# netneurolab/pypyls

Hardware: AMD Instinct MI355X
Metric: resamples/sec (perm+boot), behavioral_pls X(500x200000)/Y(500x50) fp64 (higher is better)
Workload: dtype f64

## Files before the change

pypyls_amd/csrc/plsx_compact.hip:

```cpp
#include "plsx_internal.h"

using namespace plsxi;

namespace plsxi {

template <int MT, int KT, bool TAIL = false>
int launch_xprod_cboot(plsx_ctx* ctx, int nres, int nks_c, SplitEpi se, hipStream_t st)
{
    const size_t lds = compact_lds_bytes(MT, KT, 3, nks_c, se.npairs);
    HIPCHK(set_lds(k_xprod_compact<MT, KT, 3, TAIL>, lds));
    const int ncolblk = ceil_div(ctx->Bpad, 128);
    KTimer tm(ctx, KC_XPROD, st);
    hipLaunchKernelGGL((k_xprod_compact<MT, KT, 3, TAIL>), dim3(round_up(ncolblk, 8) * round_up(nres, 8)), dim3(256),
                       lds, st, ptr<double>(ctx->Afrag_c), (size_t)nks_c * MT * 64, ptr<double>(ctx->Xc), ctx->Bpad, nks_c,
                       ptr<double>(ctx->R), ctx->Bpad, ctx->Tpp, ptr<int>(ctx->out_row_c), ptr<int>(ctx->mom_idx_c),
                       (const double*)nullptr, nres, ncolblk, se);
    LAUNCHCHK();
    return 0;
}

int launch_cboot(plsx_ctx* ctx, int nres, int nks_c, SplitEpi se, hipStream_t st)
{
    const int MTc = ceil_div(ctx->Tp, 16);
    const bool tail = ctx->Tp - (MTc - 1) * 16 <= 4 && MTc >= 2;
    switch (MTc) {
        case 1: return launch_xprod_cboot<1, 12>(ctx, nres, nks_c, se, st);
        case 2: return tail ? launch_xprod_cboot<2, 6, true>(ctx, nres, nks_c, se, st)
                            : launch_xprod_cboot<2, 6>(ctx, nres, nks_c, se, st);
        case 3: return tail ? launch_xprod_cboot<3, 4, true>(ctx, nres, nks_c, se, st)
                            : launch_xprod_cboot<3, 4>(ctx, nres, nks_c, se, st);
        case 4: return tail ? launch_xprod_cboot<4, PLSX_CKT, true>(ctx, nres, nks_c, se, st)
                            : launch_xprod_cboot<4, PLSX_CKT>(ctx, nres, nks_c, se, st);
#define PLSX_CB(M, K) case M: return tail ? launch_xprod_cboot<M, K, true>(ctx, nres, nks_c, se, st) \
                                          : launch_xprod_cboot<M, K>(ctx, nres, nks_c, se, st);
        PLSX_CB(5, 2) PLSX_CB(6, 2) PLSX_CB(7, 1) PLSX_CB(8, 1) PLSX_CB(9, 1) PLSX_CB(10, 1) PLSX_CB(11, 1) PLSX_CB(12, 1) PLSX_CB(13, 1)
#undef PLSX_CB
        default: return fail(ctx, PLSX_ERR_STATE, "compact bootstrap blocks: T' > 208");
    }
}
// ... 46 lines not shown
```

pypyls_amd/csrc/plsx_core.hip:

```cpp
#include "plsx_internal.h"
#include "plsx_resample.h"
using namespace plsxi;

namespace plsxi {

const char* const kKernelClassNames[KC_COUNT] = {"k_xprod", "k_gram", "k_small", "k_urot", "k_nt_gemm",
                                                 "k_ucorr_partial", "k_simpls_dual", "k_build_A", "k_xprod_moments",
                                                 "k_sd_cv_score", "k_sd_coef", "k_coef_prod", "k_percentile", "k_contrast"};

int plan_groups(plsx_ctx* c)
{
    c->scaled = (c->method == PLSX_BEHAVIORAL && !c->cov) ? 1 : 0;
    c->momrows = (c->method == PLSX_BEHAVIORAL && (!c->cov || c->cv_mom)) ? 1 : 0;
    const int Jw = c->momrows ? c->J : 0;
    c->gps = 0;
    c->h_slice_row0.clear(); c->h_slice_rows.clear(); c->h_slice_cell0.clear(); c->h_slice_ncell.clear();
    auto fit = [&](int mt) {
        int b = 0;
        for (int n = 1; n <= 512; ++n) {
            int td = ceil_div(n * c->Tp, 16), tw = Jw ? ceil_div(n * Jw, 16) : 0;
            if (td + 2 * tw <= mt && tw * 16 <= 48) b = n; else break;
        }
        return b;
    };
// ... 1194 lines not shown
try {
    plsx_ctx* ctx = const_cast<plsx_ctx*>(cctx);
    if (!ctx || !out || cap < 1) return PLSX_ERR_ARG;
    double ms = 0.0;
    int launches = 0;
    for (auto& ev : ctx->events) {
        if (ev.cls != KC_XPROD) continue;
        float t = 0.f;
        if (hipEventSynchronize(ev.e1) == hipSuccess && hipEventElapsedTime(&t, ev.e0, ev.e1) == hipSuccess)
            ms += t;
        ++launches;
    }
    double crows = 0.0;
    if (ctx->last_compact_n > 0) {
        std::vector<int> cnt(ctx->last_compact_n);
        if (hipMemcpy(cnt.data(), ptr<int>(ctx->rowtab_c) + (size_t)ctx->last_compact_n * ctx->last_compact_ktot,
                      cnt.size() * sizeof(int), hipMemcpyDeviceToHost) == hipSuccess) {
            for (int c : cnt) crows += 4.0 * ((std::max(c, 1) + 3) / 4);
            crows /= (double)cnt.size() * ctx->S;
        }
    }
    const bool cmp = ctx->last_compact_n > 0;
    const auto uvar = [&](int nks) { return (double)(nks > 0 && ctx->urot_tail_l ? nks + 100 : nks); };
    double vals[21] = {ms, (double)launches, (double)(cmp ? 1 : (ctx->sepmom_used ? ctx->npg_d : ctx->npg)),
                       (double)(cmp ? ceil_div(ctx->Tp, 16) : (ctx->sepmom_used ? ctx->MTd : ctx->MT)),
                       (double)ctx->Gcap * ctx->npg, (double)ctx->timed_units, (double)use_dual(ctx), crows,
                       ctx->nt_flops, (double)ctx->quad_series, (double)ctx->quad_MT, (double)ctx->quad_gpl,
                       (double)ctx->urot_waves_l, (double)ctx->urot_splits_l, (double)ctx->urot_rps_l,
                       uvar(ctx->urot_nks_first), (double)ctx->gram_chunks_l, uvar(ctx->urot_nks_last),
                       (double)ctx->gram_kind_l, (double)ctx->split_blocks_l, (double)ctx->split_reader_l};
    int n = std::min(cap, 21);
    for (int i = 0; i < n; ++i) out[i] = vals[i];
    return n;
} PLSX_CATCH(const_cast<plsx_ctx*>(cctx))

int plsx_kernel_timing(const plsx_ctx* cctx, int kernel_class, double* ms_out, int* launches_out)
try {
    plsx_ctx* ctx = const_cast<plsx_ctx*>(cctx);
    if (!ctx || kernel_class < 0 || kernel_class >= KC_COUNT) return PLSX_ERR_ARG;
    double ms = 0.0;
    int launches = 0;
    for (auto& ev : ctx->events) {
        if (ev.cls != kernel_class) continue;
        float t = 0.f;
        if (hipEventSynchronize(ev.e1) == hipSuccess && hipEventElapsedTime(&t, ev.e0, ev.e1) == hipSuccess)
            ms += t;
        ++launches;
    }
    if (ms_out) *ms_out = ms;
    if (launches_out) *launches_out = launches;
    return PLSX_OK;
} PLSX_CATCH(const_cast<plsx_ctx*>(cctx))

const char* plsx_kernel_class_name(int kernel_class)
// ... 146 lines not shown
```

pypyls_amd/csrc/plsx_internal.h:

```cpp
#pragma once
#include "plsx_kernels.h"
#include <chrono>
#include "../../include/plsx.h"

#include <algorithm>
#include <cmath>
#include <cstdio>
#include <cstdlib>
#include <cstring>
#include <new>
#include <stdexcept>
#include <string>
#include <thread>
#include <vector>

struct Buf {
    void* p = nullptr;
    size_t bytes = 0;
};

enum {
    OPT_NO_REFINE = 0, OPT_MIN_BATCH, OPT_INBLOCK_MOMENTS, OPT_NO_COMPACT_BOOT, OPT_COMPACT_BOOT_ALWAYS,
    OPT_SEPMOM_ALWAYS, OPT_NO_GRAM4, OPT_UROT_GENERIC, OPT_UROT_NO_TAIL4, OPT_NO_FIXED_X, OPT_NO_DUAL_PERM,
    OPT_TWO_PASS_BOOT, OPT_SPLIT_INBLOCK, OPT_NO_SPLIT_FUSE, OPT_SPLIT_TWO_READERS, OPT_EXPECT_RESAMPLES,
    OPT_SIMPLS_JACOBI, OPT_PERCENTILE_SORT, OPT_QUAD_SUMS, OPT_SPLIT_READER8, OPT_SIMPLS_GLOBAL,
    OPT_CROSSCOV_SPARSE, OPT_COUNT
};
static const char* const kOptionNames[OPT_COUNT] = {
    "no_refine", "min_batch", "inblock_moments", "no_compact_boot", "compact_boot_always",
    "sepmom_always", "no_gram4", "urot_generic", "urot_no_tail4", "no_fixed_x", "no_dual_perm",
    "two_pass_boot", "split_inblock", "no_split_fuse", "split_two_readers", "expect_resamples",
    "simpls_jacobi", "percentile_sort", "quad_sums", "split_reader8", "simpls_global",
    "crosscov_sparse"};

#ifndef PLSX_CKT
#define PLSX_CKT 3
#endif

struct plsx_ctx {
    int device = 0;
    std::string err;
    int opt[OPT_COUNT] = {};
    bool has_data = false, has_orig = false;
    int method = 0, S = 0, B = 0, T = 0, J = 0, n_groups = 0, n_cond = 1, mc = 0, cov = 0;
    int Tp = 0, Tpp = 0, L = 0, Kpad = 0, nks = 0, Bx = 0, Bpad = 0;
    int MT = 24, npg = 0, w0 = 0, sq0 = 0, nmom_pad = 0, scaled = 0, momrows = 0, Gcap = 0, Galloc = 0;
    int nks_t = 0, LT = 0, cv_mom = 0;
    int afrag_group0 = 0;
    int sepmom = 0, MTd = 0, npg_d = 0, sepmom_used = 0;
    size_t group_stride_d = 0;
    Buf out_row_d, mom_idx_d, Afrag_m, momn_m, scale;
    Buf Afrag_c, rank_c, rowtab_c, m1_c, m2_c, out_row_c, mom_idx_c, mask_c;
    int has_compact_maps = 0;
    size_t group_stride = 0;
    int gps = 0;
    Buf row_slice, row_local, slice_cell0, cell_momrow;
// ... 42 lines not shown
    double* keepA = nullptr;
    long long keep_cap = 0, keep_n = 0;
    Buf cichunk;
    double* vipG = nullptr;
    long long vip_cap = 0, vip_n = 0;
    int vip_c = 0;
    int cperm_active = 0, cperm_c = 0, cperm_std = 0;
    const double* cperm_obs = nullptr;
    int* cperm_count = nullptr;
    double* cperm_max = nullptr;
    long long cperm_cap = 0, cperm_n = 0;
    Buf cpA, cppart, colsd;
    bool has_okx = false, has_oky = false;
    int n_okx = 0;
    double* mom_out_arg = nullptr;
    int ncomp = 0;
    int timing = 0;
    struct TimedEv { int cls; hipEvent_t e0, e1; };
    std::vector<TimedEv> events;
    long long timed_units = 0;
    double nt_flops = 0.0;
    int quad_MT = 0, quad_gpl = 0, quad_series = 0;
    int last_compact_n = 0, last_compact_ktot = 0;
    int urot_waves_l = 0, urot_splits_l = 0, urot_rps_l = 0;
    int urot_nks_first = 0, urot_nks_last = 0, urot_tail_l = 0;
    int gram_chunks_l = 0, gram_kind_l = 0;
    double scratch_gb = 48.0;
    long long R_geom[6] = {0, 0, 0, 0, 0, 0};
    size_t R_zeroed_bytes = 0;
    double map_ms_per_gb = 0.0;
    int scratch_fixed = 0;
    double last_ms = 0.0;
    int last_launches = 0;
    void* comm = nullptr;
    int comm_rank = 0, comm_world = 1;
    int comm_team = 0;
};

namespace plsxi {


inline int fail(plsx_ctx* c, int code, const std::string& msg)
{
    if (c) c->err = msg;
    return code;
}
// ... 127 lines not shown
int run_contrast_norms(plsx_ctx* ctx, int nres, double* out_sv, hipStream_t st);
int run_contrast_fill(plsx_ctx* ctx, int nres, hipStream_t st);
int run_percentile(plsx_ctx* ctx, const double* d_data, long long nseries, int n, int i_lo, double g_lo, int i_hi,
                   double g_hi, double* d_lo, double* d_hi, hipStream_t st);
inline void coef_close(plsx_ctx* ctx)
{
    ctx->coef_active = 0; ctx->coef_n = 0;
    ctx->keepA = nullptr; ctx->keep_cap = 0; ctx->keep_n = 0;
}
inline void vip_close(plsx_ctx* ctx)
{
    ctx->vipG = nullptr; ctx->vip_cap = 0; ctx->vip_n = 0; ctx->vip_c = 0;
}
inline void cperm_close(plsx_ctx* ctx)
{
    ctx->cperm_active = 0; ctx->cperm_c = 0; ctx->cperm_std = 0;
    ctx->cperm_obs = nullptr; ctx->cperm_count = nullptr; ctx->cperm_max = nullptr;
    ctx->cperm_cap = 0; ctx->cperm_n = 0;
}
int launch_xprod(plsx_ctx* ctx, int groups, hipStream_t st);
int launch_xprod_acc(plsx_ctx* ctx, const double* Afrag, size_t gstride, int groups, int L, hipStream_t st);
int run_xprod_fixed(plsx_ctx* ctx, const int* ysrc, int nres, hipStream_t st, const double* ystack);
MomLayout moment_layout(const plsx_ctx* ctx, int npairs);
int launch_moment_blocks_raw(plsx_ctx* ctx, const MomLayout& ml, SplitEpi se, hipStream_t st);
int ensure_compact_maps(plsx_ctx* ctx);
int run_xprod(plsx_ctx* ctx, const int* xsrc, const int* ysrc, int nres, hipStream_t st,
              bool prebuilt = false, const double* ystack = nullptr, long long ystride = -1, bool sparse_rows = false);
int launch_xprod_split(plsx_ctx* ctx, int groups, SplitEpi se, hipStream_t st);
int quad_finish(plsx_ctx* ctx, double* d_usum, double* d_usq, hipStream_t st, const QuadSet* qs = nullptr);
inline int quad_blocks(int tiles) { return tiles >= 8 ? ceil_div(tiles, 8) : 1; }
int launch_cboot(plsx_ctx* ctx, int nres, int nks_c, SplitEpi se, hipStream_t st);
int launch_csplit(plsx_ctx* ctx, int m, int nks_c, SplitEpi se, hipStream_t st, bool raw = false);
int run_nt(plsx_ctx* ctx, const double* A, long long strideA, int lda, int Ma,
           const double* B1, long long strideB1, int ldb1, int N1,
           const double* B2, long long strideB2, int ldb2, int N2, int K, int batch,
           double* C1, long long strideC1, int ldc1, double* C2, long long strideC2, int ldc2,
           hipStream_t st, bool sym = false, bool accumulate = false, bool one_chunk = false);
bool nt_sym_fits(int S);
int nt_strips(plsx_ctx* ctx, const double* A, int lda, int Ma, const double* Bm, int ldb, int N, int Kc,
              double* C, int ldc, hipStream_t st, bool one_chunk = false);
int form_gram_K(plsx_ctx* ctx, const double* X, int ldx, int S, int Kc, double* K, int ldk, hipStream_t st);
int run_dual_gp(plsx_ctx* ctx, int m, int Sd, const double* ScT, int L, hipStream_t st);
int run_gram_ex(plsx_ctx* ctx, int nres, int mode, const double* E, int Erows, double* Pout,
                hipStream_t st, const double* Rsrc = nullptr);
int run_gram(plsx_ctx* ctx, int nres, bool with_p, hipStream_t st);
int run_small(plsx_ctx* ctx, SmallArgs a, int nres, hipStream_t st, const double* Rref = nullptr);
// ... 13 lines not shown
```

pypyls_amd/csrc/plsx_k_prep.h:

```cpp
#pragma once
#include "plsx_common.h"


static __global__ void k_colmean(const double* __restrict__ X, int S, int B, double* __restrict__ mean)
{
    int b = blockIdx.x * blockDim.x + threadIdx.x;
    if (b >= B) return;
    double s = 0.0;
    for (int i = 0; i < S; ++i) s += X[(size_t)i * B + b];
    mean[b] = s / (double)S;
}

static __global__ void k_center_pad(const double* __restrict__ X, const double* __restrict__ mean,
                             int S, int B, double* __restrict__ Xc, int ldx)
{
    int b = blockIdx.x * blockDim.x + threadIdx.x;
    int i = blockIdx.y;
    if (b >= B || i >= S) return;
    Xc[(size_t)i * ldx + b] = X[(size_t)i * B + b] - mean[b];
}

static __global__ void k_cell_scale(const double* __restrict__ Xc, int ldx, int B, int J,
                             const int* __restrict__ cell_start, const int* __restrict__ cell_len,
                             double* __restrict__ Xn)
// ... 21 lines not shown
struct GroupLayout {
    int n;
    int Tp;
    int J;
    int T;
    int MT;
    int w0;
    int sq0;
    int Tpp;
    int gps = 0;
    const int* row_slice = nullptr;
    const int* row_local = nullptr;
    const int* slice_cell0 = nullptr;
};

static __global__ void k_build_A_behav(const double* __restrict__ Y0, long long y_stride, int T, int S,
                                const int* __restrict__ cell_start, const int* __restrict__ cell_len,
                                const int* __restrict__ xsrc, const int* __restrict__ ysrc,
                                GroupLayout lay, int covariance, int scaled,
                                double* __restrict__ Afrag, size_t group_stride,
                                double* __restrict__ mom_n, int nmom_pad, int dense_ld = 0,
                                double* __restrict__ Amom = nullptr, size_t mom_stride = 0,
                                const int* __restrict__ rank = nullptr, int mom_pairs = PLSX_MOM_PAIRS,
                                int chain_cap = 0)
{
    extern __shared__ double sm_b[];
    const int r = blockIdx.x, j = blockIdx.y;
    const int g = r / lay.n, rr = r % lay.n;
    const double* Y = Y0 + (size_t)r * y_stride;
    const int start = cell_start[j], len = cell_len[j];
    const int* xs = xsrc ? xsrc + (size_t)r * S : nullptr;
    const int* ys = ysrc ? ysrc + (size_t)r * S : nullptr;
    double* mean = sm_b;
    double* rstd = sm_b + T;
    __shared__ int s_cnt;
    const int tid = threadIdx.x;

    if (tid == 0) {
        int c = 0;
        for (int p = start; p < start + len; ++p) c += (xs ? xs[p] : p) >= 0;
        s_cnt = c;
    }
    __syncthreads();
    const int cnt = s_cnt;
    for (int t = tid; t < T; t += blockDim.x) {
        double s = 0.0;
        for (int p = start; p < start + len; ++p) {
// ... 71 lines not shown
            double c = 0.0;
            for (int q = pl; q >= 0; q = nxt[q]) c += 1.0;
            *d0 = c; *d1 = c;
        } else if (unique) { *d0 = 1.0; *d1 = 1.0; }
        else { atomicAdd(d0, 1.0); atomicAdd(d1, 1.0); }
    };
    if (scaled && sliced) {
        const int sa = lay.row_slice[j * T], sb = lay.row_slice[j * T + T - 1];
        for (int sl = sa; sl <= sb; ++sl) {
            const size_t gg = (size_t)r * lay.gps + sl;
            double* As = Afrag + gg * group_stride;
            const int mrow = j - lay.slice_cell0[sl];
            for (int pl = tid; pl < len; pl += blockDim.x) {
                int p = start + pl;
                int xi = xs ? xs[p] : p;
                if (xi < 0) continue;
                put_weight(As + afrag_off(lay.w0 * 16 + mrow, xi, lay.MT), As + afrag_off(lay.sq0 * 16 + mrow, xi, lay.MT), pl);
            }
            if (tid == 0) mom_n[gg * nmom_pad + mrow] = (double)cnt;
        }
    } else if (scaled && Amom) {
        const int pair = r * lay.J + j;
        double* Am = Amom + (size_t)(pair / mom_pairs) * mom_stride;
        const int mrow = pair % mom_pairs, mmt = mom_pairs / 8;
        for (int pl = tid; pl < len; pl += blockDim.x) {
            int p = start + pl;
            int xi = xs ? xs[p] : p;
            if (xi < 0) continue;
            put_weight(Am + afrag_off(mrow, xi, mmt), Am + afrag_off(mom_pairs + mrow, xi, mmt), pl);
        }
        if (tid == 0) mom_n[pair] = (double)cnt;
    } else if (scaled) {
        for (int pl = tid; pl < len; pl += blockDim.x) {
            int p = start + pl;
            int xi = xs ? xs[p] : p;
            if (xi < 0) continue;
            int mrow = rr * lay.J + j;
            put_weight(A + afrag_off(lay.w0 * 16 + mrow, xi, lay.MT), A + afrag_off(lay.sq0 * 16 + mrow, xi, lay.MT), pl);
        }
        if (tid == 0) mom_n[(size_t)g * nmom_pad + rr * lay.J + j] = (double)cnt;
    }
}

static __global__ void k_build_A_mc(int S, int J, int n_cond, int mean_centering,
                             const int* __restrict__ cell_of_pos,
                             const int* __restrict__ xsrc, GroupLayout lay,
                             double* __restrict__ Afrag, size_t group_stride, int dense_ld = 0, int chain_cap = 0)
{
    extern __shared__ int sm_mc[];
    __shared__ int cnt[PLSX_MAX_CELLS];
    const int r = blockIdx.x;
    const int g = r / lay.n, rr = r % lay.n;
// ... 290 lines not shown
```

pypyls_amd/csrc/plsx_k_xprod.h:

```cpp
#pragma once
#include <type_traits>
#include <utility>

template <class F, int... I>
__device__ __forceinline__ void xprod_static_for(F&& f, std::integer_sequence<int, I...>)
{
    (f(std::integral_constant<int, I>()), ...);
}
#include "plsx_common.h"
#include "plsx_k_prep.h"

#define PLSX_RSRC_FLAGS 0x00020000
template <int NT, int PASSES, bool EVEN, int STAGE>
__device__ __forceinline__ void stage_copy_buf(const double* src, double* dst, int tid, int wave)
{
    __amdgpu_buffer_rsrc_t rs = __builtin_amdgcn_make_buffer_rsrc((void*)src, (short)0, 0x7fffffff,
                                                                   PLSX_RSRC_FLAGS);
    const int voff = tid * 16;
#pragma unroll
    for (int p = 0; p < PASSES; ++p) {
        if (EVEN || p * NT + wave * 64 < STAGE / 2) {
            __builtin_amdgcn_raw_ptr_buffer_load_lds(
                rs, (__attribute__((address_space(3))) void*)(dst + (size_t)(p * NT + wave * 64) * 2),
                16, voff, p * NT * 16, 0, 0);
// ... 96 lines not shown
            const double b = xb[s];
            const double bsq = (NSQ > 0) ? b * b : 0.0;
#pragma unroll
            for (int m = 0; m < NA; ++m)
                acc[m] = mfma_f64(sA[(s * MT + m) * 64], (m < MT - NSQ) ? b : bsq, acc[m]);
        }
#pragma unroll
        for (int s = 0; s < KT; ++s) xb[s] = xn[s];
        __syncthreads();
    };
    int kt_first = 0;
    if constexpr (EPI == 7) {
        xprod_static_for([&](auto mm) {
#pragma unroll
            for (int j = 0; j < 4 / KT; ++j) {
                const int kt = (4 / KT) * decltype(mm)::value + j;
                if (kt < nkt) pass(kt, std::integral_constant<int, decltype(mm)::value + 1>());
            }
        }, std::make_integer_sequence<int, MT>());
        kt_first = min(nkt, 4 * MT / KT);
    }
    for (int kt = kt_first; kt < nkt; ++kt) pass(kt, std::integral_constant<int, MT>());

    constexpr int W0 = MT - 2 * NSQ, SQ0 = MT - NSQ, NMOM = NSQ * 16;
    if constexpr (EPI == 6) {
        static_assert(MT == 2 * NSQ, "EPI 6 is a moment-only instantiation");
#pragma unroll
        for (int j = 0; j < NSQ; ++j)
#pragma unroll
            for (int i = 0; i < 4; ++i) {
                const int pair = grp * (NSQ * 16) + j * 16 + kq + 4 * i;
                if (pair >= se.npairs || col >= ldr) continue;
                se.scale[(size_t)pair * ldr + col] = acc[j][i];
                se.scale2[(size_t)pair * ldr + col] = acc[NSQ + j][i];
            }
        return;
    }
    if constexpr (EPI == 4) {
        static_assert(MT == 2 * NSQ, "EPI 4 is the moment-only instantiation");
#pragma unroll
        for (int j = 0; j < NSQ; ++j)
#pragma unroll
            for (int i = 0; i < 4; ++i) {
                const int pair = grp * (NSQ * 16) + j * 16 + kq + 4 * i;
                if (pair >= se.npairs || col >= ldr) continue;
                const double m1 = acc[j][i], m2 = acc[NSQ + j][i];
                const double nn = mom_n[pair];
// ... 212 lines not shown
        for (int i = 0; i < 4; ++i)
            if (orow[i] >= 0) Rg[(size_t)orow[i] * ldr] = acc[m][i] * sc[i];
    }
}

__device__ __forceinline__ d2 load_x2_buf(const double* base, int voff)
{
    __amdgpu_buffer_rsrc_t rs = __builtin_amdgcn_make_buffer_rsrc((void*)base, (short)0, 0x7fffffff, PLSX_RSRC_FLAGS);
    return __builtin_bit_cast(d2, __builtin_amdgcn_raw_buffer_load_b128(rs, voff, 0, 0));
}

__host__ __device__ constexpr int compact_stage_lds(int MT, int KT) { return ((KT * MT * 64 + 127) / 128) * 128; }
__host__ __device__ constexpr int compact_scale_regs(int KT) { return KT < 4 ? KT : 4; }
__host__ __device__ constexpr size_t compact_lds_bytes(int MT, int KT, int EPI, int nks, int J)
{
    const size_t loop = (size_t)MT * 16 * 8 + (size_t)2 * compact_stage_lds(MT, KT) * 8 + (size_t)nks * 4 * 4;
    if (EPI == 3) return loop + (J > compact_scale_regs(KT) ? (size_t)J * 128 * 8 : 0);
    const size_t epi5 = (size_t)MT * 16 * 8 + (size_t)5 * J * 128 * 8 + (size_t)MT * 16 * 5 * 8;
    return EPI == 5 && epi5 > loop ? epi5 : loop;
}

__host__ __device__ constexpr int compact_waves(int MT, int EPI, bool TAIL)
{
    if (EPI == 3) return MT > 10 ? 2 : MT == 10 ? (TAIL ? 3 : 2) : MT > 6 ? 3 : MT > 4 ? 4 : (MT == 4 && TAIL) ? 5 : 4;
    return (EPI == 5 && MT == 4 && !TAIL) ? 3 : 4;
}

template <int MT, int KT, int EPI, bool TAIL>
__global__ __launch_bounds__(256, compact_waves(MT, EPI, TAIL))
void k_xprod_compact(const double* __restrict__ Afrag, size_t group_stride,
                     const double* __restrict__ X, int ldx, int nks,
                     double* __restrict__ R, int ldr, int rows_per_group,
                     const int* __restrict__ out_row, const int* __restrict__ mom_idx,
                     const double* __restrict__ mom_n, int n_groups, int ncolblk, SplitEpi se)
{
    static_assert(EPI == 3 || EPI == 5 || EPI == 8, "compact blocks: bootstrap (3), fused split-half (5) or raw first-half sums (8)");
    extern __shared__ __attribute__((aligned(16))) double smem[];
    constexpr int NW = 4, NT = NW * 64, BC = NW * 32;
    constexpr int STAGE = KT * MT * 64;
    constexpr int STAGE_LDS = compact_stage_lds(MT, KT);
    constexpr int PASSES = (STAGE + NT * 2 - 1) / (NT * 2);
    constexpr bool EVEN = (STAGE % (NT * 2)) == 0;
    constexpr int MF = TAIL ? MT - 1 : MT;
    constexpr int NSCR = compact_scale_regs(KT);
    static_assert(MT * 16 <= NT, "the row maps are staged by one thread per row");
    const int ncb = (ncolblk + 7) & ~7;
    const int sweep = blockIdx.x / (8 * ncb);
    const int within = blockIdx.x - sweep * (8 * ncb);
    const int slot = within >> 3;
    const int grp = sweep * 8 + (slot & 7);
    const int colblk = (slot >> 3) * 8 + (within & 7);
    if (grp >= n_groups || colblk >= ncolblk) return;
    const double* Ag = Afrag + (size_t)grp * group_stride;
    const int swave = __builtin_amdgcn_readfirstlane((int)threadIdx.x >> 6);

    d4 acc0[MF > 0 ? MF : 1], acc1[MF > 0 ? MF : 1];
#pragma unroll
    for (int m = 0; m < MF; ++m) { acc0[m] = (d4){0.0, 0.0, 0.0, 0.0}; acc1[m] = (d4){0.0, 0.0, 0.0, 0.0}; }
    double tl0 = 0.0, tl1 = 0.0;

    int* s_out = reinterpret_cast<int*>(smem);
    int* s_mom = s_out + MT * 16;
    double* sStage = smem + MT * 16;
    int* s_tab = reinterpret_cast<int*>(sStage + 2 * STAGE_LDS);
    const int J3 = se.npairs;
    double* sW = reinterpret_cast<double*>(s_tab + nks * 4) + swave * (J3 * 32);
    d2 scr[NSCR];
    {
    const int tid = threadIdx.x, lane = tid & 63, wave = tid >> 6;
    const int kq = lane >> 4;
    const int cw = wave * 32 + 2 * (lane & 15);
    const int col = colblk * BC + cw;
    const bool live = col < ldr;
    const int lcol8 = (live ? col : 0) * 8;
    const int toff = (lane & 48) + (lane & 3) - lane;

    const int* tabg = se.row_tab + (size_t)grp * nks * 4;
    const int ldx8 = ldx * 8;
    int row0[KT];
#pragma unroll
    for (int s = 0; s < KT; ++s) row0[s] = tabg[s * 4 + kq];
    stage_copy_buf<NT, PASSES, EVEN, STAGE>(Ag, sStage, tid, swave);
    int orw = -1, mix = -1;
    if (tid < MT * 16) {
        orw = out_row[tid];
        if (EPI != 8) mix = mom_idx[tid];
    }
    const int ksteps = max(1, (se.row_cnt[grp] + 3) >> 2);
    const int nkt = (ksteps + KT - 1) / KT;
    const int ntab = nkt * KT * 4;
// ... 47 lines not shown
                acc1[m] = mfma_f64(a, b1, acc1[m]);
            }
            if constexpr (TAIL) {
                const double a = sT[(s * MT + MT - 1) * 64];
                tl0 = mfma_f64_4x4(a, b0, tl0);
                tl1 = mfma_f64_4x4(a, b1, tl1);
            }
        }
    };
    const int* tp = s_tab + KT * 4 + kq;
    const double* An = Ag + STAGE;
    auto pass = [&](auto curc, const d2 (&xc)[KT], d2 (&xn)[KT]) {
        constexpr int CUR = decltype(curc)::value;
        stage_copy_buf<NT, PASSES, EVEN, STAGE>(An, sStage + (CUR ^ 1) * STAGE_LDS, tid, swave);
#pragma unroll
        for (int s = 0; s < KT; ++s) xn[s] = load_x2_buf(X, tp[s * 4] + lcol8);
        An += STAGE;
        tp += KT * 4;
        contract(curc, xc, std::true_type(), KT);
        __syncthreads();
    };
    auto last = [&](int cur, const d2 (&xc)[KT]) {
#pragma unroll
        for (int j = 0; j < NSCR; ++j) scr[j] = (d2){1.0, 1.0};
        if constexpr (EPI == 3) {
            if (J3 <= NSCR) {
#pragma unroll
                for (int j = 0; j < NSCR; ++j)
                    if (j < J3)
                        scr[j] = *reinterpret_cast<const d2*>(
                            reinterpret_cast<const char*>(se.scale + ((size_t)grp * J3 + j) * ldr) + lcol8);
            } else if (live) {
                __amdgpu_buffer_rsrc_t rs = __builtin_amdgcn_make_buffer_rsrc(
                    (void*)(se.scale + (size_t)grp * J3 * ldr + colblk * BC + swave * 32), (short)0, 0x7fffffff, PLSX_RSRC_FLAGS);
                const int ln4 = __lane_id() * 4;
                for (int j = 0; j < J3; ++j)
                    __builtin_amdgcn_raw_ptr_buffer_load_lds(
                        rs, (__attribute__((address_space(3))) void*)(sW + j * 32), 4, ln4, j * ldr * 8, 0, 0);
            }
        }
        contract(cur, xc, std::false_type(), ksteps - (nkt - 1) * KT);
        if constexpr (EPI == 5) __syncthreads();
    };
    {
        std::integral_constant<int, 0> c0;
        std::integral_constant<int, 1> c1;
        int kt = 0, cur = 0;
        for (; kt + 2 < nkt; kt += 2) { pass(c0, xa, xb); pass(c1, xb, xa); }
        if (kt + 1 < nkt) {
            pass(c0, xa, xb);
#pragma unroll
            for (int s = 0; s < KT; ++s) xa[s] = xb[s];
            cur = 1;
        }
        last(cur, xa);
    }
    }

    int tid16 = threadIdx.x * 16;
    if constexpr (EPI != 5) asm volatile("" : "+v"(tid16));
    const int tid = tid16 >> 4, lane = tid & 63, wave = tid >> 6, kq = lane >> 4;
    const int cw = wave * 32 + 2 * (lane & 15), col = colblk * BC + cw;
    const bool live = col < ldr;
    auto val0 = [&](int m, int i) -> double { return (TAIL && m == MT - 1) ? tl0 : acc0[m < MF ? m : 0][i]; };
    auto val1 = [&](int m, int i) -> double { return (TAIL && m == MT - 1) ? tl1 : acc1[m < MF ? m : 0][i]; };

    if constexpr (EPI == 8) {
        if (!live) return;
        double* Rg = R + (size_t)grp * rows_per_group * ldr + col;
#pragma unroll
        for (int m = 0; m < MT; ++m)
#pragma unroll
            for (int i = 0; i < 4; ++i) {
                if (TAIL && m == MT - 1 && i > 0) break;
                const int orow = s_out[m * 16 + kq + 4 * i];
                if (orow < 0) continue;
                __builtin_nontemporal_store((d2){val0(m, i), val1(m, i)}, reinterpret_cast<d2*>(&Rg[(size_t)orow * ldr]));
            }
        return;
// ... 108 lines not shown
```

pypyls_amd/csrc/plsx_xprod.hip:

```cpp
#include "plsx_internal.h"

using namespace plsxi;

namespace plsxi {

template <int MT, int NW, int KT, int NSQ>
int launch_xprod_t(plsx_ctx* ctx, int groups, hipStream_t st)
{
    const size_t stage = (size_t)2 * (((size_t)KT * MT * 64 + 127) / 128) * 128 * 8;
    const size_t epi = (size_t)NW * 2 * NSQ * 16 * 16 * 8 + (size_t)2 * MT * 16 * 4;
    const size_t lds = std::max(stage, epi);
    HIPCHK(set_lds(k_xprod<MT, NW, KT, NSQ>, lds));
    const int ncolblk = ctx->Bpad / (NW * 16);
    dim3 grid(ncolblk * round_up(groups, 8)), block(NW * 64);
    KTimer tm(ctx, KC_XPROD, st);
    hipLaunchKernelGGL((k_xprod<MT, NW, KT, NSQ>), grid, block, lds, st,
                       ptr<double>(ctx->Afrag) + (size_t)ctx->afrag_group0 * ctx->group_stride, ctx->group_stride,
                       ptr<double>(ctx->Xc), ctx->Bpad,
                       ctx->nks, ptr<double>(ctx->R), ctx->Bpad, ctx->npg * ctx->Tpp,
                       ptr<int>(ctx->out_row), ptr<int>(ctx->mom_idx), ptr<double>(ctx->mom_n),
                       std::max(ctx->nmom_pad, 0), groups, ncolblk, ctx->mom_out_arg,
                       SplitEpi{nullptr, nullptr, nullptr, nullptr, nullptr, 0, 0}, std::max(ctx->gps, 1));
    LAUNCHCHK();
    return 0;
// ... 32 lines not shown
        hipLaunchKernelGGL((k_xprod<MT, NW, KT, 0, 2>), dim3(ncolblk * round_up(groups, 8)), dim3(NW * 64), lds, st,
                           Afrag, gstride, ptr<double>(ctx->Xc), ctx->Bpad, ctx->nks, (double*)nullptr, ctx->Bpad, 0,
                           ptr<int>(ctx->out_row_w), (const int*)nullptr, (const double*)nullptr, 0, groups, ncolblk,
                           (double*)nullptr, se, 1);
    } else {
        constexpr int NW = 4;
        const size_t lds = std::max(stage, ((size_t)2 * L + 32) * PLSX_ACC_PITCH * 8 + (size_t)MT * 16 * 4);
        HIPCHK(set_lds(k_xprod<MT, NW, KT, 0, 2>, lds));
        const int ncolblk = ctx->Bpad / (NW * 16);
        hipLaunchKernelGGL((k_xprod<MT, NW, KT, 0, 2>), dim3(ncolblk * round_up(groups, 8)), dim3(NW * 64), lds, st,
                           Afrag, gstride, ptr<double>(ctx->Xc), ctx->Bpad, ctx->nks, (double*)nullptr, ctx->Bpad, 0,
                           ptr<int>(ctx->out_row_w), (const int*)nullptr, (const double*)nullptr, 0, groups, ncolblk,
                           (double*)nullptr, se, 1);
    }
    LAUNCHCHK();
    return 0;
}

static int stage_ksteps(int nks) { return nks % 3 == 0 ? 3 : (nks % 2 == 0 ? 2 : 1); }

template <int MT, int NW, int KT, int EPI>
int launch_moments_t(plsx_ctx* ctx, size_t stride, int groups, SplitEpi se, hipStream_t st)
{
    const size_t lds = (size_t)2 * (((size_t)KT * MT * 64 + 127) / 128) * 128 * 8;
    HIPCHK(set_lds(k_xprod<MT, NW, KT, MT / 2, EPI>, lds));
    const int ncolblk = ceil_div(ctx->Bpad, NW * 16);
    hipLaunchKernelGGL((k_xprod<MT, NW, KT, MT / 2, EPI>), dim3(ncolblk * round_up(groups, 8)), dim3(NW * 64), lds, st,
                       ptr<double>(ctx->Afrag_m), stride, ptr<double>(ctx->Xc), ctx->Bpad, ctx->nks,
                       (double*)nullptr, ctx->Bpad, 0, (const int*)nullptr, (const int*)nullptr,
                       ptr<double>(ctx->momn_m), 0, groups, ncolblk, (double*)nullptr, se, 1);
    LAUNCHCHK();
    return 0;
}

template <int MT, int NW, int EPI>
int launch_moments(plsx_ctx* ctx, size_t stride, int groups, SplitEpi se, hipStream_t st)
{
    if constexpr (EPI == 4) {
        const int kt = stage_ksteps(ctx->nks);
        if (kt == 3) return launch_moments_t<MT, NW, 3, EPI>(ctx, stride, groups, se, st);
        if (kt == 2) return launch_moments_t<MT, NW, 2, EPI>(ctx, stride, groups, se, st);
    }
    return launch_moments_t<MT, NW, 1, EPI>(ctx, stride, groups, se, st);
}

template <int KT>
int launch_xprod_fixed_t(plsx_ctx* ctx, int groups, hipStream_t st)
{
    constexpr int MT = 25, NW = 4;
    const size_t stage = (size_t)2 * (((size_t)KT * MT * 64 + 127) / 128) * 128 * 8;
    const size_t lds = std::max(stage, (size_t)2 * MT * 16 * 4);
    HIPCHK(set_lds(k_xprod<MT, NW, KT, 0>, lds));
    const int ncolblk = ctx->Bpad / (NW * 16);
    dim3 grid(ncolblk * round_up(groups, 8)), block(NW * 64);
    KTimer tm(ctx, KC_XPROD, st);
    hipLaunchKernelGGL((k_xprod<MT, NW, KT, 0>), grid, block, lds, st,
                       ptr<double>(ctx->Afrag), ctx->group_stride_f, ptr<double>(ctx->Xn), ctx->Bpad,
                       ctx->nks, ptr<double>(ctx->R), ctx->Bpad, ctx->npgf * ctx->Tpp,
                       ptr<int>(ctx->out_row_f), ptr<int>(ctx->mom_idx_f), ptr<double>(ctx->mom_n), 0,
                       groups, ncolblk, (double*)nullptr, SplitEpi{nullptr, nullptr, nullptr, nullptr, nullptr, 0, 0}, 1);
    LAUNCHCHK();
// ... 78 lines not shown
        KTimer tm(ctx, KC_MOM, st);
        if (int e = launch_moments<24, 8, 4>(ctx, mstride, groups_m, se, st)) return e;
    }
    se.npairs = ctx->npg_d * ctx->J;
    se.accB = nres * ctx->Tpp;
    switch (ctx->MTd) {
        case 24: return launch_xprod_data<24>(ctx, groups_d, se, st);
        case 22: return launch_xprod_data<22>(ctx, groups_d, se, st);
        default: return launch_xprod_data<16>(ctx, groups_d, se, st);
    }
}

MomLayout moment_layout(const plsx_ctx* ctx, int npairs)
{
    const int t192 = ceil_div(npairs, 192) * 24, t128 = ceil_div(npairs, 128) * 16;
    MomLayout m;
    m.pairs = (t128 * 6 < t192 * 5) ? 128 : 192;
    m.mt = m.pairs / 8;
    m.groups = ceil_div(npairs, m.pairs);
    m.stride = (size_t)ctx->nks * m.mt * 64;
    return m;
}

template <int EPI>
int launch_moment_blocks(plsx_ctx* ctx, const MomLayout& ml, SplitEpi se, hipStream_t st)
{
    constexpr int NW = (EPI == 4) ? 8 : 4;
    KTimer tm(ctx, KC_MOM, st);
    if (ml.mt == 24) return launch_moments<24, NW, EPI>(ctx, ml.stride, ml.groups, se, st);
    return launch_moments<16, NW, EPI>(ctx, ml.stride, ml.groups, se, st);
}

int ensure_compact_maps(plsx_ctx* ctx)
{
    if (ctx->has_compact_maps) return 0;
    const int rows = ceil_div(ctx->Tp, 16) * 16;
    std::vector<int> orow(rows, -1), mrow(rows, -1);
    for (int t = 0; t < ctx->Tp; ++t) { orow[t] = t; mrow[t] = t / ctx->T; }
    if (int e = ensure(ctx, ctx->out_row_c, rows * sizeof(int))) return e;
    if (int e = ensure(ctx, ctx->mom_idx_c, rows * sizeof(int))) return e;
    HIPCHK(hipMemcpy(ctx->out_row_c.p, orow.data(), rows * sizeof(int), hipMemcpyHostToDevice));
    HIPCHK(hipMemcpy(ctx->mom_idx_c.p, mrow.data(), rows * sizeof(int), hipMemcpyHostToDevice));
    ctx->has_compact_maps = 1;
    return 0;
}

int launch_moment_blocks_raw(plsx_ctx* ctx, const MomLayout& ml, SplitEpi se, hipStream_t st)
{
    return launch_moment_blocks<6>(ctx, ml, se, st);
}

bool compact_boot_ok(const plsx_ctx* ctx)
{
    if (!(ctx->scaled && ctx->method == PLSX_BEHAVIORAL && ctx->gps == 0 && ctx->Tp <= 208 && !ctx->mom_out_arg &&
          ctx->J <= 32 && ctx->S <= 8192 && (long long)ctx->Kpad * ctx->Bpad * 8 < (1LL << 31)))
        return false;
    const int force = ctx->opt[OPT_COMPACT_BOOT_ALWAYS] ? 1 : (ctx->opt[OPT_NO_COMPACT_BOOT] ? -1 : 0);
    if (force) return force > 0;
    const int mt = ceil_div(ctx->Tp, 16);
    const double rows = (mt >= 2 && ctx->Tp - (mt - 1) * 16 <= 4) ? (mt - 1) * 16 + 4 : mt * 16;
    const double cost_c = 0.66 * 1.25 * rows / 16.0;
    const int npg_dense = ctx->sepmom ? ctx->npg_d : ctx->npg, mt_dense = ctx->sepmom ? ctx->MTd : ctx->MT;
    return cost_c * 1.1 < (double)mt_dense / npg_dense && npg_dense <= 16;
}

int run_xprod_cboot(plsx_ctx* ctx, const int* xsrc, const int* ysrc, int nres, hipStream_t st,
                    const double* ystack, long long ystride)
{
    const int S = ctx->S, J = ctx->J, MTc = ceil_div(ctx->Tp, 16), KT = MTc == 4 ? PLSX_CKT : std::max(1, 12 / MTc);
    const int nks_c = round_up(ceil_div(S, 4), KT);
    const int npairs = nres * J;
    const MomLayout ml = moment_layout(ctx, npairs);
    const int groups_m = ml.groups;
    const size_t astride = (size_t)nks_c * MTc * 64, mstride = ml.stride;
    if (int e = ensure_compact_maps(ctx)) return e;
    if (int e = ensure(ctx, ctx->Afrag_c, (size_t)nres * astride * 8 + 4096)) return e;
    if (int e = ensure(ctx, ctx->mask_c, (size_t)nres * S)) return e;
    if (int e = ensure(ctx, ctx->rank_c, (size_t)nres * S * sizeof(int))) return e;
    if (int e = ensure(ctx, ctx->rowtab_c, ((size_t)nres * nks_c * 4 + nres) * sizeof(int))) return e;
    if (int e = ensure(ctx, ctx->Afrag_m, (size_t)groups_m * mstride * 8 + 4096)) return e;
    if (int e = ensure(ctx, ctx->momn_m, (size_t)round_up(npairs, 192) * 8)) return e;
    if (int e = ensure(ctx, ctx->scale, (size_t)round_up(npairs, 8) * ctx->Bpad * 8)) return e;
    HIPCHK(hipMemsetAsync(ctx->Afrag_c.p, 0, (size_t)nres * astride * 8, st));
    HIPCHK(hipMemsetAsync(ctx->Afrag_m.p, 0, (size_t)groups_m * mstride * 8, st));
    HIPCHK(hipMemsetAsync(ctx->mask_c.p, 0, (size_t)nres * S, st));
    int* row_cnt = ptr<int>(ctx->rowtab_c) + (size_t)nres * nks_c * 4;
    ctx->last_compact_n = nres; ctx->last_compact_ktot = nks_c * 4;
    {
        KTimer tm(ctx, KC_BUILD, st);
        hipLaunchKernelGGL(k_drawn_mask, dim3(ceil_div(S, 256), nres), dim3(256), 0, st, xsrc, S, ptr<uint8_t>(ctx->mask_c));
        LAUNCHCHK();
        hipLaunchKernelGGL(k_split_rank, dim3(nres), dim3(64), 0, st, ptr<uint8_t>(ctx->mask_c), S, nks_c * 4,
                           ptr<int>(ctx->rank_c), ptr<int>(ctx->rowtab_c), row_cnt);
        LAUNCHCHK();
        GroupLayout lay;
        lay.n = 1; lay.Tp = ctx->Tp; lay.J = J; lay.T = ctx->T; lay.MT = MTc; lay.w0 = MTc; lay.sq0 = MTc; lay.Tpp = ctx->Tpp;
        int cap = 0;
        const size_t blds = build_lds_behav(ctx, &cap);
        hipLaunchKernelGGL(k_build_A_behav, dim3(nres, J), dim3(256), blds, st,
                           ystack ? ystack : ptr<double>(ctx->Y), ystack ? ystride : 0LL, ctx->T, S,
                           ptr<int>(ctx->cell_start), ptr<int>(ctx->cell_len), xsrc, ysrc, lay, ctx->cov, 1,
                           ptr<double>(ctx->Afrag_c), astride, ptr<double>(ctx->momn_m), 0, 0,
                           ptr<double>(ctx->Afrag_m), mstride, ptr<int>(ctx->rank_c), ml.pairs, cap);
        LAUNCHCHK();
    }
    SplitEpi se;
    memset(&se, 0, sizeof(se));
    se.scale = ptr<double>(ctx->scale);
    se.npairs = npairs;
    if (int e = launch_moment_blocks<4>(ctx, ml, se, st)) return e;
    se.npairs = J;
    se.accB = nres * ctx->Tpp;
    se.row_tab = ptr<int>(ctx->rowtab_c);
    se.row_cnt = row_cnt;
    return launch_cboot(ctx, nres, nks_c, se, st);
}

int run_xprod(plsx_ctx* ctx, const int* xsrc, const int* ysrc, int nres, hipStream_t st,
              bool prebuilt, const double* ystack, long long ystride, bool sparse_rows)
{
    if (ystride < 0) ystride = (long long)ctx->S * ctx->T;
    const int groups = ceil_div(nres, ctx->npg);
    if (int e = ensure_scratch(ctx, groups)) return e;
    if (ctx->timing) ctx->timed_units += nres;
    const int pgroups = phys_groups(ctx, groups);
    ctx->last_compact_n = 0;
    if (prebuilt) return launch_xprod(ctx, pgroups, st);
    if (sparse_rows && xsrc && compact_boot_ok(ctx)) return run_xprod_cboot(ctx, xsrc, ysrc, nres, st, ystack, ystride);
    if (ctx->sepmom && ctx->method == PLSX_BEHAVIORAL && !ctx->mom_out_arg) {
        const long long cost_a = (long long)groups * ctx->MT;
        const long long cost_b = (long long)ceil_div(nres, ctx->npg_d) * ctx->MTd +
                                 (long long)ceil_div(nres * ctx->J, PLSX_MOM_PAIRS) * 24;
        const bool force_b = ctx->opt[OPT_SEPMOM_ALWAYS] != 0;
// ... 129 lines not shown
```

pypyls_amd/engine.py:

```python
import ctypes
import threading
import os

import numpy as np

from . import _build

_LIB = None

PLSX_BEHAVIORAL = 0
PLSX_MEANCENTERED = 1
PLSX_REGRESSION = 2
PLSX_FLAG_COVARIANCE = 1


class PlsxError(RuntimeError):
    pass


def _load():
    global _LIB
    if _LIB is not None:
        return _LIB
    import torch
# ... 812 lines not shown
        self._check(self.lib.plsx_set_timing(self.ctx, 1 if enable else 0))

    def kernel_timing(self):
        out = {}
        k = 0
        while True:
            name = self.lib.plsx_kernel_class_name(k)
            if not name:
                break
            ms, n = ctypes.c_double(), ctypes.c_int()
            self._check(self.lib.plsx_kernel_timing(self.ctx, k, ctypes.byref(ms), ctypes.byref(n)))
            if n.value:
                out[name.decode()] = (ms.value, n.value)
            k += 1
        return out

    def set_perm_path(self, dual):
        rc = self.lib.plsx_set_perm_path(self.ctx, -1 if dual is None else (1 if dual else 0))
        if rc < 0:
            self._check(rc)
        return bool(rc)

    def last_timing(self):
        buf = (ctypes.c_double * 21)()
        n = self.lib.plsx_last_timing(self.ctx, buf, 21)
        keys = ['xprod_ms', 'xprod_launches', 'resamples_per_group', 'm_tiles', 'superbatch',
                'xprod_resamples', 'dual_perm', 'compact_row_fraction', 'nt_flops', 'quad_series', 'quad_m_tiles',
                'quad_blocks_per_lv', 'urot_waves', 'urot_splits', 'urot_res_per_split', 'urot_variant',
                'gram_chunks', 'urot_variant_last', 'gram_kernel', 'split_blocks', 'split_reader']
        return {k: buf[i] for i, k in enumerate(keys[:max(n, 0)])}


_DEFAULT = {}
_DEFAULT_LOCK = threading.Lock()


def default_engine(device=None, replica=0):
    torch = _torch()
    if device is None:
        device = torch.cuda.current_device() if torch.cuda.is_available() else 0
    key = (int(device), int(replica))
    with _DEFAULT_LOCK:
        eng = _DEFAULT.get(key)
        if eng is None or not getattr(eng, 'ctx', None):
            if not _DEFAULT:
                import atexit
                atexit.register(release_default_engine)
            eng = _DEFAULT[key] = Engine(device=key[0])
    return eng


IDLE_RELEASE_S = 300.0
# ... 47 lines not shown
```

Measured before the change: 6050.

## Fold first-moment sums into compact bootstrap xprod padding rows

When the compact bootstrap tile has spare padding rows, the per-LV weights are written into those rows of the main A fragment, so the cross-product kernel also produces the first moments (sum of X). The separate moment pass then only computes X^2 sums through a new EPI 9 variant with half the rows, and the compact kernel's epilogue computes the standard deviation scale in registers from the shuffled first moments and the counts. This removes half of the moment GEMM work and its traffic, at the cost of extra epilogue shuffles and changed wave counts for MT=2.

After: 6112 (median of 6 runs). 1.01x the previous value.

```diff
diff --git a/pypyls_amd/csrc/plsx_compact.hip b/pypyls_amd/csrc/plsx_compact.hip
--- a/pypyls_amd/csrc/plsx_compact.hip
+++ b/pypyls_amd/csrc/plsx_compact.hip
@@ -7,6 +7,7 @@
 template <int MT, int KT, bool TAIL = false>
 int launch_xprod_cboot(plsx_ctx* ctx, int nres, int nks_c, SplitEpi se, hipStream_t st)
 {
+    se.nmu = compact_moment_rows(ctx) ? ctx->Tp : 0;
     const size_t lds = compact_lds_bytes(MT, KT, 3, nks_c, se.npairs);
     HIPCHK(set_lds(k_xprod_compact<MT, KT, 3, TAIL>, lds));
     const int ncolblk = ceil_div(ctx->Bpad, 128);
@@ -14,7 +15,7 @@
     hipLaunchKernelGGL((k_xprod_compact<MT, KT, 3, TAIL>), dim3(round_up(ncolblk, 8) * round_up(nres, 8)), dim3(256),
                        lds, st, ptr<double>(ctx->Afrag_c), (size_t)nks_c * MT * 64, ptr<double>(ctx->Xc), ctx->Bpad, nks_c,
                        ptr<double>(ctx->R), ctx->Bpad, ctx->Tpp, ptr<int>(ctx->out_row_c), ptr<int>(ctx->mom_idx_c),
-                       (const double*)nullptr, nres, ncolblk, se);
+                       ptr<double>(ctx->momn_m), nres, ncolblk, se);
     LAUNCHCHK();
     return 0;
 }
diff --git a/pypyls_amd/csrc/plsx_core.hip b/pypyls_amd/csrc/plsx_core.hip
--- a/pypyls_amd/csrc/plsx_core.hip
+++ b/pypyls_amd/csrc/plsx_core.hip
@@ -1240,14 +1240,15 @@
     }
     const bool cmp = ctx->last_compact_n > 0;
     const auto uvar = [&](int nks) { return (double)(nks > 0 && ctx->urot_tail_l ? nks + 100 : nks); };
-    double vals[21] = {ms, (double)launches, (double)(cmp ? 1 : (ctx->sepmom_used ? ctx->npg_d : ctx->npg)),
+    double vals[22] = {ms, (double)launches, (double)(cmp ? 1 : (ctx->sepmom_used ? ctx->npg_d : ctx->npg)),
                        (double)(cmp ? ceil_div(ctx->Tp, 16) : (ctx->sepmom_used ? ctx->MTd : ctx->MT)),
                        (double)ctx->Gcap * ctx->npg, (double)ctx->timed_units, (double)use_dual(ctx), crows,
                        ctx->nt_flops, (double)ctx->quad_series, (double)ctx->quad_MT, (double)ctx->quad_gpl,
                        (double)ctx->urot_waves_l, (double)ctx->urot_splits_l, (double)ctx->urot_rps_l,
                        uvar(ctx->urot_nks_first), (double)ctx->gram_chunks_l, uvar(ctx->urot_nks_last),
-                       (double)ctx->gram_kind_l, (double)ctx->split_blocks_l, (double)ctx->split_reader_l};
-    int n = std::min(cap, 21);
+                       (double)ctx->gram_kind_l, (double)ctx->split_blocks_l, (double)ctx->split_reader_l,
+                       (double)(cmp && ctx->last_moment_rows ? 1 : 0)};
+    int n = std::min(cap, 22);
     for (int i = 0; i < n; ++i) out[i] = vals[i];
     return n;
 } PLSX_CATCH(const_cast<plsx_ctx*>(cctx))
diff --git a/pypyls_amd/csrc/plsx_internal.h b/pypyls_amd/csrc/plsx_internal.h
--- a/pypyls_amd/csrc/plsx_internal.h
+++ b/pypyls_amd/csrc/plsx_internal.h
@@ -24,14 +24,14 @@
     OPT_SEPMOM_ALWAYS, OPT_NO_GRAM4, OPT_UROT_GENERIC, OPT_UROT_NO_TAIL4, OPT_NO_FIXED_X, OPT_NO_DUAL_PERM,
     OPT_TWO_PASS_BOOT, OPT_SPLIT_INBLOCK, OPT_NO_SPLIT_FUSE, OPT_SPLIT_TWO_READERS, OPT_EXPECT_RESAMPLES,
     OPT_SIMPLS_JACOBI, OPT_PERCENTILE_SORT, OPT_QUAD_SUMS, OPT_SPLIT_READER8, OPT_SIMPLS_GLOBAL,
-    OPT_CROSSCOV_SPARSE, OPT_COUNT
+    OPT_CROSSCOV_SPARSE, OPT_NO_MOMENT_ROWS, OPT_COUNT
 };
 static const char* const kOptionNames[OPT_COUNT] = {
     "no_refine", "min_batch", "inblock_moments", "no_compact_boot", "compact_boot_always",
     "sepmom_always", "no_gram4", "urot_generic", "urot_no_tail4", "no_fixed_x", "no_dual_perm",
     "two_pass_boot", "split_inblock", "no_split_fuse", "split_two_readers", "expect_resamples",
     "simpls_jacobi", "percentile_sort", "quad_sums", "split_reader8", "simpls_global",
-    "crosscov_sparse"};
+    "crosscov_sparse", "no_moment_rows"};
 
 #ifndef PLSX_CKT
 #define PLSX_CKT 3
@@ -120,6 +120,7 @@
     double nt_flops = 0.0;
     int quad_MT = 0, quad_gpl = 0, quad_series = 0;
     int last_compact_n = 0, last_compact_ktot = 0;
+    int last_moment_rows = 0;
     int urot_waves_l = 0, urot_splits_l = 0, urot_rps_l = 0;
     int urot_nks_first = 0, urot_nks_last = 0, urot_tail_l = 0;
     int gram_chunks_l = 0, gram_kind_l = 0;
@@ -293,6 +294,9 @@
 int launch_xprod_acc(plsx_ctx* ctx, const double* Afrag, size_t gstride, int groups, int L, hipStream_t st);
 int run_xprod_fixed(plsx_ctx* ctx, const int* ysrc, int nres, hipStream_t st, const double* ystack);
 MomLayout moment_layout(const plsx_ctx* ctx, int npairs);
+MomLayout moment2_layout(const plsx_ctx* ctx, int npairs);
+int compact_boot_ksteps(int mt);
+bool compact_moment_rows(const plsx_ctx* ctx);
 int launch_moment_blocks_raw(plsx_ctx* ctx, const MomLayout& ml, SplitEpi se, hipStream_t st);
 int ensure_compact_maps(plsx_ctx* ctx);
 int run_xprod(plsx_ctx* ctx, const int* xsrc, const int* ysrc, int nres, hipStream_t st,
diff --git a/pypyls_amd/csrc/plsx_k_prep.h b/pypyls_amd/csrc/plsx_k_prep.h
--- a/pypyls_amd/csrc/plsx_k_prep.h
+++ b/pypyls_amd/csrc/plsx_k_prep.h
@@ -67,7 +67,7 @@
                                 double* __restrict__ mom_n, int nmom_pad, int dense_ld = 0,
                                 double* __restrict__ Amom = nullptr, size_t mom_stride = 0,
                                 const int* __restrict__ rank = nullptr, int mom_pairs = PLSX_MOM_PAIRS,
-                                int chain_cap = 0)
+                                int chain_cap = 0, int mom_row0 = -1)
 {
     extern __shared__ double sm_b[];
     const int r = blockIdx.x, j = blockIdx.y;
@@ -185,12 +185,15 @@
     } else if (scaled && Amom) {
         const int pair = r * lay.J + j;
         double* Am = Amom + (size_t)(pair / mom_pairs) * mom_stride;
-        const int mrow = pair % mom_pairs, mmt = mom_pairs / 8;
+        const int mrow = pair % mom_pairs, mmt = mom_row0 >= 0 ? mom_pairs / 16 : mom_pairs / 8;
         for (int pl = tid; pl < len; pl += blockDim.x) {
             int p = start + pl;
             int xi = xs ? xs[p] : p;
             if (xi < 0) continue;
-            put_weight(Am + afrag_off(mrow, xi, mmt), Am + afrag_off(mom_pairs + mrow, xi, mmt), pl);
+            if (mom_row0 >= 0)
+                put_weight(A + afrag_off(mom_row0 + j, rank[(size_t)r * S + xi], lay.MT), Am + afrag_off(mrow, xi, mmt), pl);
+            else
+                put_weight(Am + afrag_off(mrow, xi, mmt), Am + afrag_off(mom_pairs + mrow, xi, mmt), pl);
         }
         if (tid == 0) mom_n[pair] = (double)cnt;
     } else if (scaled) {
diff --git a/pypyls_amd/csrc/plsx_k_xprod.h b/pypyls_amd/csrc/plsx_k_xprod.h
--- a/pypyls_amd/csrc/plsx_k_xprod.h
+++ b/pypyls_amd/csrc/plsx_k_xprod.h
@@ -142,7 +142,19 @@
     }
     for (int kt = kt_first; kt < nkt; ++kt) pass(kt, std::integral_constant<int, MT>());
 
-    constexpr int W0 = MT - 2 * NSQ, SQ0 = MT - NSQ, NMOM = NSQ * 16;
+    constexpr int W0 = (EPI == 9) ? 0 : MT - 2 * NSQ, SQ0 = MT - NSQ, NMOM = NSQ * 16;
+    if constexpr (EPI == 9) {
+        static_assert(MT == NSQ, "EPI 9 runs every tile against X^2");
+#pragma unroll
+        for (int j = 0; j < MT; ++j)
+#pragma unroll
+            for (int i = 0; i < 4; ++i) {
+                const int pair = grp * (MT * 16) + j * 16 + kq + 4 * i;
+                if (pair >= se.npairs || col >= ldr) continue;
+                se.scale[(size_t)pair * ldr + col] = acc[j][i];
+            }
+        return;
+    }
     if constexpr (EPI == 6) {
         static_assert(MT == 2 * NSQ, "EPI 6 is a moment-only instantiation");
 #pragma unroll
@@ -401,6 +413,7 @@
 
 __host__ __device__ constexpr int compact_waves(int MT, int EPI, bool TAIL)
 {
+    if (EPI == 3 && MT == 2) return TAIL ? 7 : 6;
     if (EPI == 3) return MT > 10 ? 2 : MT == 10 ? (TAIL ? 3 : 2) : MT > 6 ? 3 : MT > 4 ? 4 : (MT == 4 && TAIL) ? 5 : 4;
     return (EPI == 5 && MT == 4 && !TAIL) ? 3 : 4;
 }
@@ -445,6 +458,8 @@
     const int J3 = se.npairs;
     double* sW = reinterpret_cast<double*>(s_tab + nks * 4) + swave * (J3 * 32);
     d2 scr[NSCR];
+    const int mrow0 = (EPI == 3) ? se.nmu : 0;
+    int cnt_lo[NSCR], cnt_hi[NSCR];
     {
     const int tid = threadIdx.x, lane = tid & 63, wave = tid >> 6;
     const int kq = lane >> 4;
@@ -538,9 +553,18 @@
     };
     auto last = [&](int cur, const d2 (&xc)[KT]) {
 #pragma unroll
-        for (int j = 0; j < NSCR; ++j) scr[j] = (d2){1.0, 1.0};
+        for (int j = 0; j < NSCR; ++j) { scr[j] = (d2){1.0, 1.0}; cnt_lo[j] = 0; cnt_hi[j] = 0; }
         if constexpr (EPI == 3) {
             if (J3 <= NSCR) {
+                if (mrow0 > 0) {
+#pragma unroll
+                    for (int j = 0; j < NSCR; ++j)
+                        if (j < J3) {
+                            const double v = mom_n[(size_t)grp * J3 + j];
+                            cnt_lo[j] = __builtin_amdgcn_readfirstlane(__double2loint(v));
+                            cnt_hi[j] = __builtin_amdgcn_readfirstlane(__double2hiint(v));
+                        }
+                }
 #pragma unroll
                 for (int j = 0; j < NSCR; ++j)
                     if (j < J3)
@@ -571,6 +595,36 @@
         }
         last(cur, xa);
     }
+    }
+
+    if constexpr (EPI == 3) {
+        if (mrow0 > 0 && J3 <= NSCR) {
+            const int ln = __lane_id();
+            const bool second = (ln & 16) != 0;
+#pragma unroll
+            for (int j = 0; j < NSCR; ++j) {
+                if (j >= J3) continue;
+                const int r = mrow0 + j;
+                double a0, a1;
+                if constexpr (TAIL) { a0 = tl0; a1 = tl1; }
+                else {
+                    const int ri = (r & 15) >> 2;
+                    a0 = acc0[MT - 1][0]; a1 = acc1[MT - 1][0];
+#pragma unroll
+                    for (int q = 1; q < 4; ++q)
+                        if (ri == q) { a0 = acc0[MT - 1][q]; a1 = acc1[MT - 1][q]; }
+                }
+                const int src = ((r & 3) << 4) | (ln & 15);
+                const double nn = __hiloint2double(cnt_hi[j], cnt_lo[j]);
+                const double m1x = __shfl(a0, src), m1y = __shfl(a1, src);
+                const double m1 = second ? m1y : m1x, m2 = second ? scr[j].y : scr[j].x;
+                const double var = (m2 - m1 * m1 / nn) / (nn - 1.0);
+                double sc = (var > 0.0) ? sd_rsqrt(var) : 0.0;
+                asm volatile("" : "+v"(sc));
+                const double other = __shfl_xor(sc, 16);
+                scr[j] = second ? (d2){other, sc} : (d2){sc, other};
+            }
+        }
     }
 
     int tid16 = threadIdx.x * 16;
diff --git a/pypyls_amd/csrc/plsx_xprod.hip b/pypyls_amd/csrc/plsx_xprod.hip
--- a/pypyls_amd/csrc/plsx_xprod.hip
+++ b/pypyls_amd/csrc/plsx_xprod.hip
@@ -78,10 +78,11 @@
 template <int MT, int NW, int KT, int EPI>
 int launch_moments_t(plsx_ctx* ctx, size_t stride, int groups, SplitEpi se, hipStream_t st)
 {
+    constexpr int NSQ = (EPI == 9) ? MT : MT / 2;
     const size_t lds = (size_t)2 * (((size_t)KT * MT * 64 + 127) / 128) * 128 * 8;
-    HIPCHK(set_lds(k_xprod<MT, NW, KT, MT / 2, EPI>, lds));
+    HIPCHK(set_lds(k_xprod<MT, NW, KT, NSQ, EPI>, lds));
     const int ncolblk = ceil_div(ctx->Bpad, NW * 16);
-    hipLaunchKernelGGL((k_xprod<MT, NW, KT, MT / 2, EPI>), dim3(ncolblk * round_up(groups, 8)), dim3(NW * 64), lds, st,
+    hipLaunchKernelGGL((k_xprod<MT, NW, KT, NSQ, EPI>), dim3(ncolblk * round_up(groups, 8)), dim3(NW * 64), lds, st,
                        ptr<double>(ctx->Afrag_m), stride, ptr<double>(ctx->Xc), ctx->Bpad, ctx->nks,
                        (double*)nullptr, ctx->Bpad, 0, (const int*)nullptr, (const int*)nullptr,
                        ptr<double>(ctx->momn_m), 0, groups, ncolblk, (double*)nullptr, se, 1);
@@ -92,7 +93,7 @@
 template <int MT, int NW, int EPI>
 int launch_moments(plsx_ctx* ctx, size_t stride, int groups, SplitEpi se, hipStream_t st)
 {
-    if constexpr (EPI == 4) {
+    if constexpr (EPI == 4 || EPI == 9) {
         const int kt = stage_ksteps(ctx->nks);
         if (kt == 3) return launch_moments_t<MT, NW, 3, EPI>(ctx, stride, groups, se, st);
         if (kt == 2) return launch_moments_t<MT, NW, 2, EPI>(ctx, stride, groups, se, st);
@@ -217,10 +218,21 @@
     return m;
 }
 
+MomLayout moment2_layout(const plsx_ctx* ctx, int npairs)
+{
+    const int t384 = ceil_div(npairs, 384) * 24, t256 = ceil_div(npairs, 256) * 16;
+    MomLayout m;
+    m.pairs = (t256 * 6 < t384 * 5) ? 256 : 384;
+    m.mt = m.pairs / 16;
+    m.groups = ceil_div(npairs, m.pairs);
+    m.stride = (size_t)ctx->nks * m.mt * 64;
+    return m;
+}
+
 template <int EPI>
 int launch_moment_blocks(plsx_ctx* ctx, const MomLayout& ml, SplitEpi se, hipStream_t st)
 {
-    constexpr int NW = (EPI == 4) ? 8 : 4;
+    constexpr int NW = (EPI == 6) ? 4 : 8;
     KTimer tm(ctx, KC_MOM, st);
     if (ml.mt == 24) return launch_moments<24, NW, EPI>(ctx, ml.stride, ml.groups, se, st);
     return launch_moments<16, NW, EPI>(ctx, ml.stride, ml.groups, se, st);
@@ -259,13 +271,25 @@
     return cost_c * 1.1 < (double)mt_dense / npg_dense && npg_dense <= 16;
 }
 
+int compact_boot_ksteps(int mt) { return mt == 4 ? PLSX_CKT : std::max(1, 12 / mt); }
+
+bool compact_moment_rows(const plsx_ctx* ctx)
+{
+    if (ctx->opt[OPT_NO_MOMENT_ROWS]) return false;
+    const int mt = ceil_div(ctx->Tp, 16);
+    const bool tail = mt >= 2 && ctx->Tp - (mt - 1) * 16 <= 4;
+    const int rows = tail ? (mt - 1) * 16 + 4 : mt * 16;
+    return ctx->J <= compact_scale_regs(compact_boot_ksteps(mt)) && rows - ctx->Tp >= ctx->J;
+}
+
 int run_xprod_cboot(plsx_ctx* ctx, const int* xsrc, const int* ysrc, int nres, hipStream_t st,
                     const double* ystack, long long ystride)
 {
-    const int S = ctx->S, J = ctx->J, MTc = ceil_div(ctx->Tp, 16), KT = MTc == 4 ? PLSX_CKT : std::max(1, 12 / MTc);
+    const int S = ctx->S, J = ctx->J, MTc = ceil_div(ctx->Tp, 16), KT = compact_boot_ksteps(MTc);
     const int nks_c = round_up(ceil_div(S, 4), KT);
     const int npairs = nres * J;
-    const MomLayout ml = moment_layout(ctx, npairs);
+    const bool mrows = compact_moment_rows(ctx);
+    const MomLayout ml = mrows ? moment2_layout(ctx, npairs) : moment_layout(ctx, npairs);
     const int groups_m = ml.groups;
     const size_t astride = (size_t)nks_c * MTc * 64, mstride = ml.stride;
     if (int e = ensure_compact_maps(ctx)) return e;
@@ -274,13 +298,13 @@
     if (int e = ensure(ctx, ctx->rank_c, (size_t)nres * S * sizeof(int))) return e;
     if (int e = ensure(ctx, ctx->rowtab_c, ((size_t)nres * nks_c * 4 + nres) * sizeof(int))) return e;
     if (int e = ensure(ctx, ctx->Afrag_m, (size_t)groups_m * mstride * 8 + 4096)) return e;
-    if (int e = ensure(ctx, ctx->momn_m, (size_t)round_up(npairs, 192) * 8)) return e;
+    if (int e = ensure(ctx, ctx->momn_m, (size_t)round_up(npairs, 384) * 8)) return e;
     if (int e = ensure(ctx, ctx->scale, (size_t)round_up(npairs, 8) * ctx->Bpad * 8)) return e;
     HIPCHK(hipMemsetAsync(ctx->Afrag_c.p, 0, (size_t)nres * astride * 8, st));
     HIPCHK(hipMemsetAsync(ctx->Afrag_m.p, 0, (size_t)groups_m * mstride * 8, st));
     HIPCHK(hipMemsetAsync(ctx->mask_c.p, 0, (size_t)nres * S, st));
     int* row_cnt = ptr<int>(ctx->rowtab_c) + (size_t)nres * nks_c * 4;
-    ctx->last_compact_n = nres; ctx->last_compact_ktot = nks_c * 4;
+    ctx->last_compact_n = nres; ctx->last_compact_ktot = nks_c * 4; ctx->last_moment_rows = mrows ? 1 : 0;
     {
         KTimer tm(ctx, KC_BUILD, st);
         hipLaunchKernelGGL(k_drawn_mask, dim3(ceil_div(S, 256), nres), dim3(256), 0, st, xsrc, S, ptr<uint8_t>(ctx->mask_c));
@@ -296,14 +320,14 @@
                            ystack ? ystack : ptr<double>(ctx->Y), ystack ? ystride : 0LL, ctx->T, S,
                            ptr<int>(ctx->cell_start), ptr<int>(ctx->cell_len), xsrc, ysrc, lay, ctx->cov, 1,
                            ptr<double>(ctx->Afrag_c), astride, ptr<double>(ctx->momn_m), 0, 0,
-                           ptr<double>(ctx->Afrag_m), mstride, ptr<int>(ctx->rank_c), ml.pairs, cap);
+                           ptr<double>(ctx->Afrag_m), mstride, ptr<int>(ctx->rank_c), ml.pairs, cap, mrows ? ctx->Tp : -1);
         LAUNCHCHK();
     }
     SplitEpi se;
     memset(&se, 0, sizeof(se));
     se.scale = ptr<double>(ctx->scale);
     se.npairs = npairs;
-    if (int e = launch_moment_blocks<4>(ctx, ml, se, st)) return e;
+    if (int e = mrows ? launch_moment_blocks<9>(ctx, ml, se, st) : launch_moment_blocks<4>(ctx, ml, se, st)) return e;
     se.npairs = J;
     se.accB = nres * ctx->Tpp;
     se.row_tab = ptr<int>(ctx->rowtab_c);
diff --git a/pypyls_amd/engine.py b/pypyls_amd/engine.py
--- a/pypyls_amd/engine.py
+++ b/pypyls_amd/engine.py
@@ -858,12 +858,13 @@
         return bool(rc)
 
     def last_timing(self):
-        buf = (ctypes.c_double * 21)()
-        n = self.lib.plsx_last_timing(self.ctx, buf, 21)
+        buf = (ctypes.c_double * 22)()
+        n = self.lib.plsx_last_timing(self.ctx, buf, 22)
         keys = ['xprod_ms', 'xprod_launches', 'resamples_per_group', 'm_tiles', 'superbatch',
                 'xprod_resamples', 'dual_perm', 'compact_row_fraction', 'nt_flops', 'quad_series', 'quad_m_tiles',
                 'quad_blocks_per_lv', 'urot_waves', 'urot_splits', 'urot_res_per_split', 'urot_variant',
-                'gram_chunks', 'urot_variant_last', 'gram_kernel', 'split_blocks', 'split_reader']
+                'gram_chunks', 'urot_variant_last', 'gram_kernel', 'split_blocks', 'split_reader',
+                'moment_rows']
         return {k: buf[i] for i, k in enumerate(keys[:max(n, 0)])}
 
 
```
